# JonathonLuiten/PReMVOS

Hardware: AMD Instinct MI355X
Metric: frames/sec (proposal+refine+flow) on 480p DAVIS frames (higher is better)
Workload: dtype f32

## Files before the change

premvos_amd/_lib.py:

```python
from __future__ import annotations

import ctypes as C
import os

import torch

from . import build as _build

_LIB = None
ABI_VERSION = 21

ACT_NONE, ACT_RELU, ACT_LEAKY, ACT_SIGMOID = 0, 1, 2, 3
MASK_BBOX_SLABS = 16
ACT_SPLIT8_BF16 = 0x200
OUT_NHWC, OUT_PIXSHUF2 = 0, 1
PREC_F32, PREC_BF16, PREC_BF16X3 = 0, 1, 3
PRECISIONS = {"fp32": PREC_F32, "bf16": PREC_BF16, "bf16x3": PREC_BF16X3}


class ConvDesc(C.Structure):
    _fields_ = [
        ("inp", C.c_void_p), ("wgt", C.c_void_p), ("bias", C.c_void_p), ("res", C.c_void_p),
        ("out", C.c_void_p),
        ("n", C.c_int32), ("h", C.c_int32), ("w", C.c_int32), ("cin", C.c_int32),
# ... 96 lines not shown
    "premvos_track_gt_scores_f64": [_vp, _vp, _vp, _i32, _i32, _vp, C.c_double, _vp, _vp, _vp, _vp, _vp, _vp],
    "premvos_track_combine_f64": [_vp, _i32, _i32, _i32, _vp, C.c_int64, _vp, _i32, _vp, _vp, _vp, _vp, _vp, _vp, _vp],
    "premvos_viz_scores_u8": [_vp, _i32, _i32, _vp, _vp, _i32, _vp, _vp, C.c_int64, _vp, _i32, _vp, _vp, C.c_int64, _vp, _vp],
    "premvos_reid_max_distance_f64": [_vp, _i32, _vp, C.c_int64, _vp, _vp, _vp],
    "premvos_davis_counts_u8":[_vp, _vp, _i32, _i32, _i32, _vp, _i32, _i32, _vp, _vp, _vp],
    "premvos_bits_overlap_i32": [_vp, _i32, C.c_int64, C.c_int64, _vp, _vp, _i32, _vp, C.c_int64, _vp, C.c_int64, _vp],
    "premvos_prewarp_reid_f64": [_vp, _vp, _i32, _i32, _vp, _vp, _i32, _vp, _vp, _vp, _vp, _vp],
    "premvos_prewarp_chain_f64": [_vp, C.c_int64, _vp, C.c_int64, _vp, _vp, _vp, _vp, _vp, _vp, _i32, _i32, _vp, _vp, _vp, _vp, _i32, _vp, _vp,
                                  _vp, _vp],
    "premvos_prewarp_paint_bits_u8": [_vp, _i32, C.c_int64, C.c_int64, _vp, _vp, _vp, _vp, _vp, _i32, _vp, _vp, _i32, _i32, _i32, _vp, _vp,
                                      _i32, _vp, _vp],
    "premvos_prewarp_negatives_i32": [_vp, _i32, C.c_int64, C.c_int64, _i32, _i32, _i32, _i32, _vp, _i32, _vp, _vp, _vp, _vp],
    "premvos_prewarp_gather_neg_u8": [_vp, _i32, C.c_int64, _i32, _i32, _i32, _i32, _vp, _vp, _vp, _vp],
    "premvos_prewarp_chain_neg_f64": [_vp, C.c_int64, _vp, C.c_int64, _vp, _vp, _vp, _vp, _vp, _vp, _i32, _i32, _i32, _vp, _vp, _vp, _vp, _i32,
                                      _vp, _vp, _vp, _vp],
    "premvos_prewarp_paint_neg_bits_u8": [_vp, _i32, C.c_int64, C.c_int64, _vp, _vp, _vp, _vp, _vp, _i32, _vp, _vp, _i32, _i32, _i32, _i32, _vp,
                                          _vp, _i32, _vp, _vp],
    "premvos_mask_warp_pack_bits_u8": [_vp, _i32, _i32, _i32, _vp, _vp, _vp, _vp, _vp, _i32, _i32, _vp, _vp, C.c_int64, _vp],
    "premvos_idmap_vote_u8": [_vp, _i32, C.c_int64, C.c_int64, _vp, _vp, _vp, _vp],
    "premvos_crf_unary_labels_f32": [_vp, _i32, _i32, _i32, _i32, _f32, _vp, _vp, _vp, _vp],
    "premvos_crf_norm_f32": [_vp, _i32, _i32, _i32, _f32, _f32, _i32, _vp, _vp],
    "premvos_crf_step_f32": [_vp, _vp, _vp, _vp, _vp, _i32, _i32, _i32, _i32, _f32, _i32, _f32, _f32, _f32, _i32, _f32, _vp, _vp],
    "premvos_crf_argmax_u8": [_vp, _i32, _i32, _i32, _i32, _vp, _vp, _vp, _vp],
}


POST_SIGNATURES = {
    "premvos_cc_dilate_u8": [_vp, _i32, _i32, _i32, _i32, _i32, _vp, _vp],
    "premvos_cc_label_i32": [_vp, C.c_int64, _i32, _i32, _vp, _vp],
    "premvos_cc_keep_largest_u8": [_vp, _vp, _i32, _i32, _i32, _i32, _vp, _vp, _vp, _vp, _vp],
}


class FrameFiles(C.Structure):
    _fields_ = [("flo_path", C.c_char_p), ("flow", C.c_void_p), ("flow_row_stride", C.c_int64), ("h", C.c_int32), ("w", C.c_int32),
                ("boxes", C.c_void_p * 2), ("probs", C.c_void_p * 2), ("count", C.c_int32 * 2), ("scale", C.c_float),
                ("json_path", C.c_char_p * 4), ("conf", C.c_void_p), ("rle_pool", C.c_void_p), ("rle_offsets", C.c_void_p)]


class PremvosError(RuntimeError):
    pass


def lib_path() -> str:
    return _build.LIB


def load():
    global _LIB
    if _LIB is not None:
        return _LIB
    path = _build.LIB
    stale = None
    try:
        if _build.needs_build():
            import fcntl
            with open(os.path.join(os.path.dirname(path), ".build.lock"), "w") as lock:
                fcntl.flock(lock, fcntl.LOCK_EX)
                if _build.needs_build():
                    _build.build_lib()
    except Exception as e:
        if not os.path.exists(path):
            raise PremvosError(
                f"libpremvos_hip.so is missing and could not be built ({e}); the HIP path has no fallback") from e
        stale = e
    lib = C.CDLL(path)
    lib.premvos_last_error.restype = C.c_char_p
    lib.premvos_last_error.argtypes = []
    lib.premvos_abi_version.restype = C.c_int
    lib.premvos_abi_version.argtypes = []
    if lib.premvos_abi_version() != ABI_VERSION:
        raise PremvosError(f"{path} has ABI version {lib.premvos_abi_version()}, this package binds version {ABI_VERSION}"
                           + (f" (rebuilding failed: {stale})" if stale else "") + "; rebuild with python -m premvos_amd.build")
    if stale is not None:
        import warnings
        warnings.warn(f"libpremvos_hip.so is older than its sources and could not be rebuilt ({stale}); using it as is")
    for name, argtypes in list(SIGNATURES.items()) + list(POST_SIGNATURES.items()):
        fn = getattr(lib, name)
        fn.argtypes = argtypes
        fn.restype = C.c_int
    lib.premvos_conv2d_workspace_bytes.argtypes = [C.POINTER(ConvDesc)]
    lib.premvos_conv2d_workspace_bytes.restype = C.c_int64
    lib.premvos_crc32c_host.argtypes = [_vp, C.c_int64]
    lib.premvos_crc32c_host.restype = C.c_uint32
    lib.premvos_refine_output_workspace_bytes.argtypes = [_i32, _i32, _i32, _i32]
    lib.premvos_refine_output_workspace_bytes.restype = C.c_int64
    lib.premvos_rle_counts_to_string_host.argtypes = [_vp, C.c_int64, _vp, C.c_int64]
    lib.premvos_rle_counts_to_string_host.restype = C.c_int64
    lib.premvos_rle_strings_host.argtypes = [_vp, _vp, _i32, C.c_int64, _vp, C.c_int64, _vp]
    lib.premvos_rle_strings_host.restype = C.c_int64
    lib.premvos_write_frame_files_host.argtypes = [C.POINTER(FrameFiles)]
    lib.premvos_write_frame_files_host.restype = C.c_int
    lib.premvos_format_floats_host.argtypes = [_vp, C.c_int64, _i32, _vp, C.c_int64]
    lib.premvos_format_floats_host.restype = C.c_int
    lib.premvos_rle_workspace_bytes.argtypes = [_i32, _i32, _i32]
    lib.premvos_rle_workspace_bytes.restype = C.c_int64
    lib.premvos_jpeg_workspace_bytes.argtypes = [_vp]
    lib.premvos_jpeg_workspace_bytes.restype = C.c_int64
    lib.premvos_dwconv3x3_variant.argtypes = [_i32] * 10
    lib.premvos_dwconv3x3_variant.restype = C.c_int
    _LIB = lib
    return lib


def check(rc: int, what: str = ""):
    if rc != 0:
        raise PremvosError(f"{what} failed ({rc}): {load().premvos_last_error().decode()}")


def current_stream() -> int:
# ... 16 lines not shown
```

premvos_amd/csrc/refine_ops.hip:

```cpp
#include "common.h"

#pragma clang fp contract(off)

namespace {

inline int grid_for(long total, int per_block = 256, int cap = 1 << 22) {
  long g = (total + per_block - 1) / per_block;
  return (int)(g < 1 ? 1 : g > cap ? cap : g);
}

__device__ inline void tf_lerp(int d, float scale, int in_size, int* lo, int* hi, float* t) {
  const float s = (float)d * scale;
  const float f = floorf(s);
  *lo = (int)f;
  const int c = (int)ceilf(s);
  *hi = c < in_size - 1 ? c : in_size - 1;
  *t = s - f;
}

__global__ __launch_bounds__(256) void refine_input_kernel(const uint8_t* __restrict__ frame, int H, int W,
                                                           const float* __restrict__ boxes,
                                                           const int* __restrict__ count, int P, int S,
                                                           float* __restrict__ out, int* __restrict__ crops) {
  const long total = (long)P * S * S;
  const float mean[3] = {0.485f, 0.456f, 0.406f}, stdv[3] = {0.229f, 0.224f, 0.225f};
  const int n = *count < P ? *count : P;
  for (long idx = (long)blockIdx.x * 256 + threadIdx.x; idx < total; idx += (long)gridDim.x * 256) {
    const int x = idx % S, y = (idx / S) % S, p = idx / ((long)S * S);
    float4 o = make_float4(0.f, 0.f, 0.f, 0.f);
    if (p < n) {
      const float* b = boxes + p * 4;
      const int by0 = (int)rintf(b[0]), bx0 = (int)rintf(b[1]), by1 = (int)rintf(b[2]), bx1 = (int)rintf(b[3]);
      const int cy0 = by0 - 50 > 0 ? by0 - 50 : 0, cx0 = bx0 - 50 > 0 ? bx0 - 50 : 0;
// ... 217 lines not shown
        if constexpr (PRE_RELU)
          v[cx] = make_float4(ok ? fmaxf(t.x, 0.f) : 0.f, ok ? fmaxf(t.y, 0.f) : 0.f, ok ? fmaxf(t.z, 0.f) : 0.f, ok ? fmaxf(t.w, 0.f) : 0.f);
        else
          v[cx] = make_float4(ok ? t.x : 0.f, ok ? t.y : 0.f, ok ? t.z : 0.f, ok ? t.w : 0.f);
      }
#pragma unroll
      for (int o = 0; o < TR; ++o) {
        const int kj = j - o * STRIDE;
        if (kj < 0 || kj > 2) continue;
#pragma unroll
        for (int q = 0; q < TW; ++q)
#pragma unroll
          for (int i = 0; i < 3; ++i) {
            const float4 a = v[q * STRIDE + i], kk = k[kj * 3 + i];
            acc[o][q].x += a.x * kk.x; acc[o][q].y += a.y * kk.y; acc[o][q].z += a.z * kk.z; acc[o][q].w += a.w * kk.w;
          }
        if (kj == 2 && oy0 + o * dil < ho) {
          float* orow = out + (((long)b * ho + oy0 + o * dil) * wo) * out_ps;
#pragma unroll
          for (int q = 0; q < TW; ++q) {
            if (ox0 + q * dil >= wo) break;
            float4 r = acc[o][q];
            if ((act & 0xff) == PREMVOS_ACT_RELU) {
              r.x = fmaxf(r.x, 0.f); r.y = fmaxf(r.y, 0.f); r.z = fmaxf(r.z, 0.f); r.w = fmaxf(r.w, 0.f);
            }
            store_unit(orow + (long)(ox0 + q * dil) * out_ps, cg, r, act);
          }
        }
      }
    }
  }
}

__global__ __launch_bounds__(256) void resize_bilinear_kernel(const float* __restrict__ in, int in_ps, int n, int h,
                                                              int w, int c4, float* __restrict__ out, int out_ps,
                                                              int ho, int wo, int align) {
  const long total = (long)n * ho * wo * c4;
  const float sy = (align && ho > 1) ? (float)(h - 1) / (float)(ho - 1) : (float)h / (float)ho;
  const float sx = (align && wo > 1) ? (float)(w - 1) / (float)(wo - 1) : (float)w / (float)wo;
  for (long idx = (long)blockIdx.x * 256 + threadIdx.x; idx < total; idx += (long)gridDim.x * 256) {
    const int cg = idx % c4;
    const long pix = idx / c4;
    const int ox = pix % wo, oy = (pix / wo) % ho, b = pix / ((long)wo * ho);
    int ylo, yhi, xlo, xhi;
    float ty, tx;
    tf_lerp(oy, sy, h, &ylo, &yhi, &ty);
    tf_lerp(ox, sx, w, &xlo, &xhi, &tx);
    const float* base = in + (long)b * h * w * in_ps + cg * 4;
    const float4 tl = *reinterpret_cast<const float4*>(base + ((long)ylo * w + xlo) * in_ps);
    const float4 tr = *reinterpret_cast<const float4*>(base + ((long)ylo * w + xhi) * in_ps);
    const float4 bl = *reinterpret_cast<const float4*>(base + ((long)yhi * w + xlo) * in_ps);
    const float4 br = *reinterpret_cast<const float4*>(base + ((long)yhi * w + xhi) * in_ps);
    float4 o;
    float top, bot;
    top = tl.x + (tr.x - tl.x) * tx; bot = bl.x + (br.x - bl.x) * tx; o.x = top + (bot - top) * ty;
    top = tl.y + (tr.y - tl.y) * tx; bot = bl.y + (br.y - bl.y) * tx; o.y = top + (bot - top) * ty;
    top = tl.z + (tr.z - tl.z) * tx; bot = bl.z + (br.z - bl.z) * tx; o.z = top + (bot - top) * ty;
    top = tl.w + (tr.w - tl.w) * tx; bot = bl.w + (br.w - bl.w) * tx; o.w = top + (bot - top) * ty;
    *reinterpret_cast<float4*>(out + pix * out_ps + cg * 4) = o;
  }
}

__global__ __launch_bounds__(256) void broadcast_kernel(const float* __restrict__ in, int in_ps, int n, int hw, int c4,
                                                        float* __restrict__ out, int out_ps) {
  const long total = (long)n * hw * c4;
  for (long idx = (long)blockIdx.x * 256 + threadIdx.x; idx < total; idx += (long)gridDim.x * 256) {
    const int cg = idx % c4;
    const long pix = idx / c4;
    const int b = pix / hw;
    *reinterpret_cast<float4*>(out + pix * out_ps + cg * 4) =
        *reinterpret_cast<const float4*>(in + (long)b * in_ps + cg * 4);
  }
}

__global__ __launch_bounds__(256) void seg_softmax_kernel(const float* __restrict__ logits, int ps, int P, int lh,
                                                          int lw, int S, float* __restrict__ prob,
                                                          uint8_t* __restrict__ cls) {
  const long total = (long)P * S * S;
  const float sy = (float)lh / (float)S, sx = (float)lw / (float)S;
  for (long idx = (long)blockIdx.x * 256 + threadIdx.x; idx < total; idx += (long)gridDim.x * 256) {
    const int x = idx % S, y = (idx / S) % S, p = idx / ((long)S * S);
    int ylo, yhi, xlo, xhi;
    float ty, tx;
    tf_lerp(y, sy, lh, &ylo, &yhi, &ty);
    tf_lerp(x, sx, lw, &xlo, &xhi, &tx);
    const float* base = logits + (long)p * lh * lw * ps;
    float l[2];
    for (int ch = 0; ch < 2; ++ch) {
      const float tl = base[((long)ylo * lw + xlo) * ps + ch], tr = base[((long)ylo * lw + xhi) * ps + ch];
      const float bl = base[((long)yhi * lw + xlo) * ps + ch], br = base[((long)yhi * lw + xhi) * ps + ch];
      const float top = tl + (tr - tl) * tx, bot = bl + (br - bl) * tx;
      l[ch] = top + (bot - top) * ty;
// ... 253 lines not shown
#define PV_DW_ROW(PR, ST)                                                                                                   \
  hipLaunchKernelGGL((dwconv3x3_row_kernel<PR, ST, 4>), g, dim3(256), 0, s, in, in_ps, n, h, w, c4, wgt, bias, out, out_ps, ho, wo, \
                     pt, pl, act, c_pad)
    if (v.pre_relu && v.stride == 1) PV_DW_ROW(true, 1);
    else if (v.pre_relu) PV_DW_ROW(true, 2);
    else if (v.stride == 1) PV_DW_ROW(false, 1);
    else PV_DW_ROW(false, 2);
#undef PV_DW_ROW
    return premvos::check_launch("dwconv3x3_row");
  }
  const long total = (long)n * ho * wo * c4;
  if (v.pre_relu)
    hipLaunchKernelGGL(dwconv3x3_kernel<true>, dim3(grid_for(total)), dim3(256), 0, s, in, in_ps, n, h, w, c4,
                       wgt, bias, out, out_ps, ho, wo, stride, dilation, pt, pl, act, c_pad);
  else
    hipLaunchKernelGGL(dwconv3x3_kernel<false>, dim3(grid_for(total)), dim3(256), 0, s, in, in_ps, n, h, w, c4,
                       wgt, bias, out, out_ps, ho, wo, stride, dilation, pt, pl, act, c_pad);
  return premvos::check_launch("dwconv3x3");
}

extern "C" int premvos_resize_bilinear_f32(const float* in, int32_t in_ps, int32_t n, int32_t h, int32_t w, int32_t c,
                                           float* out, int32_t out_ps, int32_t ho, int32_t wo, int32_t align_corners,
                                           void* stream) {
  PV_REQUIRE(in && out, "resize_bilinear: null pointer");
  PV_REQUIRE(n > 0 && h > 0 && w > 0 && c > 0 && ho > 0 && wo > 0, "resize_bilinear: bad dims");
  PV_REQUIRE(c % 4 == 0 && in_ps % 4 == 0 && out_ps % 4 == 0 && in_ps >= c && out_ps >= c,
             "resize_bilinear: C and strides must be multiples of 4");
  PV_REQUIRE(premvos::aligned16(in) && premvos::aligned16(out), "resize_bilinear: pointers must be 16-byte aligned");
  hipLaunchKernelGGL(resize_bilinear_kernel, dim3(grid_for((long)n * ho * wo * (c / 4))), dim3(256), 0,
                     static_cast<hipStream_t>(stream), in, in_ps, n, h, w, c / 4, out, out_ps, ho, wo, align_corners);
  return premvos::check_launch("resize_bilinear");
}

extern "C" int premvos_broadcast_pixel_f32(const float* in, int32_t in_ps, int32_t n, int32_t c, float* out,
                                           int32_t out_ps, int32_t h, int32_t w, void* stream) {
  PV_REQUIRE(in && out, "broadcast_pixel: null pointer");
  PV_REQUIRE(n > 0 && c > 0 && h > 0 && w > 0, "broadcast_pixel: bad dims");
  PV_REQUIRE(c % 4 == 0 && in_ps % 4 == 0 && out_ps % 4 == 0 && in_ps >= c && out_ps >= c,
             "broadcast_pixel: C and strides must be multiples of 4");
  PV_REQUIRE(premvos::aligned16(in) && premvos::aligned16(out), "broadcast_pixel: pointers must be 16-byte aligned");
  hipLaunchKernelGGL(broadcast_kernel, dim3(grid_for((long)n * h * w * (c / 4))), dim3(256), 0,
                     static_cast<hipStream_t>(stream), in, in_ps, n, h * w, c / 4, out, out_ps);
  return premvos::check_launch("broadcast_pixel");
}

extern "C" int64_t premvos_refine_output_workspace_bytes(int32_t max_boxes, int32_t size, int32_t h, int32_t w) {
  const long nblk = ((long)h * w + UNCROP_PIX - 1) / UNCROP_PIX;
  return (int64_t)max_boxes * size * size * (sizeof(float) + 1) + (int64_t)max_boxes * nblk * sizeof(double) + 256;
}

namespace {

struct OutputWorkspace {
  double* partial;
  float* prob;
  uint8_t* cls;
  int nblk;
};

inline OutputWorkspace output_workspace(void* workspace, int max_boxes, int size, int h, int w) {
  OutputWorkspace o;
  o.nblk = (int)(((long)h * w + UNCROP_PIX - 1) / UNCROP_PIX);
  char* ws = static_cast<char*>(workspace);
  o.partial = reinterpret_cast<double*>(ws);
  o.prob = reinterpret_cast<float*>(ws + (((long)max_boxes * o.nblk * sizeof(double) + 255) / 256) * 256);
  o.cls = reinterpret_cast<uint8_t*>(o.prob + (long)max_boxes * size * size);
// ... 71 lines not shown
```

premvos_amd/refinement/model.py:

```python
from __future__ import annotations

import os
from typing import Dict, List, Optional, Tuple

import torch

from .. import _lib, arena, ops
from ..ops import ACT_NONE, ACT_RELU, NHWC
from ..plan import LaunchPlan
from . import tta as tta_mod

INPUT_SIZE = 385
EPS_BACKBONE, EPS_HEAD = 1e-3, 1e-5
ATROUS_RATES = (6, 12, 18)
BLOCKS = (
    ("entry_flow/block1", (128, 128, 128), "conv", False, 1, 2),
    ("entry_flow/block2", (256, 256, 256), "conv", False, 1, 2),
    ("entry_flow/block3", (728, 728, 728), "conv", False, 1, 2),
    ("middle_flow/block1", (728, 728, 728), "sum", False, 16, 1),
    ("exit_flow/block1", (728, 1024, 1024), "conv", False, 1, 2),
    ("exit_flow/block2", (1536, 1536, 2048), "none", True, 1, 1),
)
DECODER_SKIP = "entry_flow/block2/unit_1/xception_module/separable_conv2"

# ... 54 lines not shown
        def alloc(n, h, w, c) -> NHWC:
            ps = (c + 3) // 4 * 4
            return NHWC(A.alloc(n, h, w, ps, "f32", pooled=ps == c), c=c)

        def release(v: Optional[NHWC]):
            if v is not None:
                A.release(v)

        split_pw = net.precision == "bf16x3" and os.environ.get("PREMVOS_BF16X3_SPLIT", "1") != "0"
        self.split_pw = split_pw
        S8 = net.packed_s8

        def alloc_s8(n, h, w, c) -> NHWC:
            assert c % 8 == 0
            return NHWC(A.alloc(n, h, w, c, "s8"), c=c, layout="s8")

        scope = {"tag": ""}

        def conv(x, name, out, out_s8=None, **kw):
            self.conv(scope["tag"] + name, x, (S8 if x.layout == "s8" else PK)[name], out, out_s8, **kw)

        def dwconv(x: NHWC, name: str, out: NHWC, stride=1, rate=1, pre_relu=False, act=ACT_NONE):
            k = DW[name]
            assert x.c == k.c and out.c == k.c and x.layout == "f32"
            flags = act | (_lib.ACT_SPLIT8_BF16 if out.layout == "s8" else 0)

            def f(x=x, out=out, k=k):
                _lib.check(lib.premvos_dwconv3x3_f32(x.ptr, x.ps, x.n, x.h, x.w, x.c, k.wgt.data_ptr(),
                                                     k.bias.data_ptr(), k.c_pad, out.ptr, out.ps, out.h, out.w, stride,
                                                     rate, rate, rate, int(pre_relu), flags, _lib.current_stream()),
                           "dwconv3x3")
            self.add(f"dw:{scope['tag']}{name}", f)
            self.dw_bytes[f"dw:{scope['tag']}{name}"] = 4.0 * k.c * (x.n * x.h * x.w + out.n * out.h * out.w)

        def alloc_mid(n, h, w, c, name=None):
            return alloc_s8(n, h, w, c) if split_pw and (name is None or name in S8) else alloc(n, h, w, c)

        S = INPUT_SIZE
        self.frames = A.side((G, H, W, 3), torch.uint8)
        NG = 1 if packed else G
        self.boxes_g = A.side((NG, PF, 4), torch.float32)
        self.count = A.side((G,), torch.int32)
        self.crops = A.side((NG, PF, 4), torch.int32)
        self.frame, self.boxes = self.frames[0], self.boxes_g[0]
        self.net_in = alloc(P, S, S, 4)

        def mk_input():
            if packed:
                for g, off, n in self.layout:
                    _lib.check(lib.premvos_refine_input_u8(self.frames[g].data_ptr(), H, W, self.boxes_g[0, off:].data_ptr(),
                                                           self.count[g:].data_ptr(), n, S, self.net_in.images(off, n).ptr,
                                                           self.crops[0, off:].data_ptr(), _lib.current_stream()), "refine_input")
                return
            for g in range(G):
                _lib.check(lib.premvos_refine_input_u8(self.frames[g].data_ptr(), H, W, self.boxes_g[g].data_ptr(),
                                                       self.count[g:].data_ptr(), PF, S,
                                                       self.net_in.images(g * PF, PF).ptr, self.crops[g].data_ptr(),
                                                       _lib.current_stream()), "refine_input")
        self.add("refine_input", mk_input)

        def body(net_in: NHWC, P: int, S: int, tag: str = "", named: bool = True) -> NHWC:
            scope["tag"] = tag
            h1 = ops.out_size(S, 3, 2, 1, 1)
            c11 = alloc(P, h1, h1, 32)
            conv(net_in, "entry_flow/conv1_1", c11, stride=(2, 2), pad=(1, 1), act=ACT_RELU)
            if net_in is not self.net_in:
# ... 41 lines not shown
                        if f"{prefix}/separable_conv{i}" == DECODER_SKIP:
                            skip_feat = cur
                        else:
                            release(cur)
                    cur = o
                if sc is not None:
                    release(sc)
                release(inp)
                x = cur
            feat = x
            if named:
                self.xception_out = feat
            fh = feat.h

            cat = alloc_mid(P, fh, fh, 1280)
            cat8 = cat.layout == "s8"
            gp = alloc(P, 1, 1, 2048)
            self.add(tag + "gap", lambda i=feat, o=gp: _lib.check(lib.premvos_global_avgpool_f32(
                i.ptr, i.ps, i.n, i.h * i.w, i.c, o.ptr, o.ps, _lib.current_stream()), "gap"))
            ip = alloc(P, 1, 1, 256)
            conv(gp, "image_pooling", ip, act=ACT_RELU)
            release(gp)
            bc = alloc(P, fh, fh, 256) if cat8 else cat.slice(0, 256)
            self.add(tag + "broadcast", lambda i=ip, o=bc: _lib.check(lib.premvos_broadcast_pixel_f32(
                i.ptr, i.ps, i.n, 256, o.ptr, o.ps, o.h, o.w, _lib.current_stream()), "broadcast"))
            release(ip)
            if cat8:
                self.add(f"split8:{tag}image_pooling", lambda i=bc, o=cat.slice(0, 256): ops.split8(i, o))
                release(bc)
                conv(x8, "aspp0", None, cat.slice(256, 256), act=ACT_RELU)
                release(x8)
            else:
                conv(feat, "aspp0", cat.slice(256, 256), act=ACT_RELU)
            for i, r in enumerate(ATROUS_RATES, 1):
                t = alloc_mid(P, fh, fh, 2048)
                dwconv(feat, f"aspp{i}_depthwise", t, rate=r, act=ACT_RELU)
                if cat8:
                    conv(t, f"aspp{i}_pointwise", None, cat.slice(256 * (i + 1), 256), act=ACT_RELU)
                else:
                    conv(t, f"aspp{i}_pointwise", cat.slice(256 * (i + 1), 256), act=ACT_RELU)
                release(t)
            if not named:
                release(feat)
            aspp = alloc(P, fh, fh, 256)
            conv(cat, "concat_projection", aspp, act=ACT_RELU)
            release(cat)
            if named:
                self.aspp_out = aspp

            dh = int((float(S) - 1.0) * 0.25 + 1.0)
            assert skip_feat is not None and skip_feat.h == dh
            dcat = alloc(P, dh, dh, 304)
            self.add(tag + "resize_aspp", lambda i=aspp, o=dcat.slice(0, 256): _lib.check(lib.premvos_resize_bilinear_f32(
                i.ptr, i.ps, i.n, i.h, i.w, 256, o.ptr, o.ps, o.h, o.w, 1, _lib.current_stream()), "resize"))
            if not named:
                release(aspp)
            conv(skip_feat, "decoder/feature_projection0", dcat.slice(256, 48), act=ACT_RELU)
            release(skip_feat)
            d = dcat
            for j in (0, 1):
                t = alloc_mid(P, dh, dh, d.c, f"decoder/decoder_conv{j}_pointwise")
                dwconv(d, f"decoder/decoder_conv{j}_depthwise", t, act=ACT_RELU)
                release(d)
                o = alloc(P, dh, dh, 256)
                conv(t, f"decoder/decoder_conv{j}_pointwise", o, act=ACT_RELU)
                release(t)
                d = o
            logits = alloc(P, dh, dh, 2)
            conv(d, "logits/features", logits)
            if named:
                self.decoder_out = d
            else:
                release(d)
            scope["tag"] = ""
            return logits

        tta = net.tta
        self.member_logits: List[NHWC] = []
        if tta is None:
            self.logits = body(self.net_in, P, S)
            self.member_logits.append(self.logits)
        else:
            self.logits = None
            nb = 2 if tta.flip else 1
            for scale in tta.scales:
                Ss, L = tta_mod.scale_dimension(S, scale), tta_mod.scale_dimension(S, max(1.0, scale) / 4.0)
                if Ss == S and nb == 1:
                    x = self.net_in
                else:
                    x = alloc(P * nb, Ss, Ss, 4)
                    self.add(f"tta_input:{Ss}", lambda o=x, Ss=Ss: _lib.check(lib.premvos_refine_tta_input_f32(
                        self.net_in.ptr, P, S, o.ptr, Ss, nb - 1, _lib.current_stream()), "refine_tta_input"))
                lg = body(x, P * nb, Ss, tag=f"tta{Ss}/", named=False)
                if lg.h != L:
                    assert lg.h < L and lg.ps == 4
# ... 160 lines not shown
```

Before: 54.26.

## Fuse ASPP atrous depthwise convs and decoder upsample into depthwise kernels

Adds a multirate depthwise kernel that computes all three ASPP atrous depthwise convolutions in one pass over the feature map, plus a lattice variant for small maps. It also adds a decoder depthwise kernel that bilinearly upsamples the ASPP output on the fly instead of writing a resized tensor first. The aim is fewer launches and less global memory traffic on the refinement network tail. In exchange it adds new code paths, higher register pressure, and all three ASPP temporaries must be live at the same time.

```diff
diff --git a/include/premvos_refine_hip.h b/include/premvos_refine_hip.h
--- /dev/null
+++ b/include/premvos_refine_hip.h
@@ -0,0 +1,21 @@
+#ifndef PREMVOS_REFINE_HIP_H
+#define PREMVOS_REFINE_HIP_H
+
+#include <stdint.h>
+
+#ifdef __cplusplus
+extern "C" {
+#endif
+
+int premvos_dwconv3x3_upsrc_f32(const float* src, int32_t src_ps, int32_t hs, int32_t ws, int32_t c_up, const float* in, int32_t in_ps,
+                                int32_t n, int32_t h, int32_t w, int32_t c, const float* wgt, const float* bias, int32_t c_pad, float* out,
+                                int32_t out_ps, int32_t act, void* stream);
+
+int premvos_dwconv3x3_multirate_f32(const float* in, int32_t in_ps, int32_t n, int32_t h, int32_t w, int32_t c, int32_t c_pad,
+                                    int32_t n_rates, const int32_t* rates, const float* const* wgt, const float* const* bias,
+                                    float* const* out, const int32_t* out_ps, int32_t act, void* stream);
+
+#ifdef __cplusplus
+}
+#endif
+#endif
diff --git a/premvos_amd/_lib.py b/premvos_amd/_lib.py
--- a/premvos_amd/_lib.py
+++ b/premvos_amd/_lib.py
@@ -152,6 +152,18 @@
 }
 
 
+REFINE_SIGNATURES = {
+    "premvos_dwconv3x3_upsrc_f32": [_vp, _i32, _i32, _i32, _i32, _vp, _i32, _i32, _i32, _i32, _i32, _vp, _vp, _i32, _vp, _i32, _i32, _vp],
+    "premvos_dwconv3x3_multirate_f32": [_vp, _i32, _i32, _i32, _i32, _i32, _i32, _i32, _vp, _vp, _vp, _vp, _vp, _i32, _vp],
+}
+
+
+def multirate_args(rates, wgts, biases, outs, out_ps):
+    n = len(rates)
+    assert 1 <= n <= 3 and len(wgts) == len(biases) == len(outs) == len(out_ps) == n
+    return ((C.c_int32 * n)(*rates), (C.c_void_p * n)(*wgts), (C.c_void_p * n)(*biases), (C.c_void_p * n)(*outs), (C.c_int32 * n)(*out_ps))
+
+
 class FrameFiles(C.Structure):
     _fields_ = [("flo_path", C.c_char_p), ("flow", C.c_void_p), ("flow_row_stride", C.c_int64), ("h", C.c_int32), ("w", C.c_int32),
                 ("boxes", C.c_void_p * 2), ("probs", C.c_void_p * 2), ("count", C.c_int32 * 2), ("scale", C.c_float),
@@ -195,7 +207,7 @@
     if stale is not None:
         import warnings
         warnings.warn(f"libpremvos_hip.so is older than its sources and could not be rebuilt ({stale}); using it as is")
-    for name, argtypes in list(SIGNATURES.items()) + list(POST_SIGNATURES.items()):
+    for name, argtypes in list(SIGNATURES.items()) + list(POST_SIGNATURES.items()) + list(REFINE_SIGNATURES.items()):
         fn = getattr(lib, name)
         fn.argtypes = argtypes
         fn.restype = C.c_int
diff --git a/premvos_amd/csrc/refine_ops.hip b/premvos_amd/csrc/refine_ops.hip
--- a/premvos_amd/csrc/refine_ops.hip
+++ b/premvos_amd/csrc/refine_ops.hip
@@ -1,4 +1,7 @@
+#include <utility>
+
 #include "common.h"
+#include "../../include/premvos_refine_hip.h"
 
 #pragma clang fp contract(off)
 
@@ -282,12 +285,24 @@
   }
 }
 
+__device__ __forceinline__ float resize_scale(int in_size, int out_size, int align) {
+  return (align && out_size > 1) ? (float)(in_size - 1) / (float)(out_size - 1) : (float)in_size / (float)out_size;
+}
+
+__device__ __forceinline__ float4 lerp4(const float4 a, const float4 b, const float t) {
+  return make_float4(a.x + (b.x - a.x) * t, a.y + (b.y - a.y) * t, a.z + (b.z - a.z) * t, a.w + (b.w - a.w) * t);
+}
+
+__device__ __forceinline__ float4 bilerp4(const float4 tl, const float4 tr, const float4 bl, const float4 br, const float tx,
+                                          const float ty) {
+  return lerp4(lerp4(tl, tr, tx), lerp4(bl, br, tx), ty);
+}
+
 __global__ __launch_bounds__(256) void resize_bilinear_kernel(const float* __restrict__ in, int in_ps, int n, int h,
                                                               int w, int c4, float* __restrict__ out, int out_ps,
                                                               int ho, int wo, int align) {
   const long total = (long)n * ho * wo * c4;
-  const float sy = (align && ho > 1) ? (float)(h - 1) / (float)(ho - 1) : (float)h / (float)ho;
-  const float sx = (align && wo > 1) ? (float)(w - 1) / (float)(wo - 1) : (float)w / (float)wo;
+  const float sy = resize_scale(h, ho, align), sx = resize_scale(w, wo, align);
   for (long idx = (long)blockIdx.x * 256 + threadIdx.x; idx < total; idx += (long)gridDim.x * 256) {
     const int cg = idx % c4;
     const long pix = idx / c4;
@@ -301,13 +316,298 @@
     const float4 tr = *reinterpret_cast<const float4*>(base + ((long)ylo * w + xhi) * in_ps);
     const float4 bl = *reinterpret_cast<const float4*>(base + ((long)yhi * w + xlo) * in_ps);
     const float4 br = *reinterpret_cast<const float4*>(base + ((long)yhi * w + xhi) * in_ps);
-    float4 o;
-    float top, bot;
-    top = tl.x + (tr.x - tl.x) * tx; bot = bl.x + (br.x - bl.x) * tx; o.x = top + (bot - top) * ty;
-    top = tl.y + (tr.y - tl.y) * tx; bot = bl.y + (br.y - bl.y) * tx; o.y = top + (bot - top) * ty;
-    top = tl.z + (tr.z - tl.z) * tx; bot = bl.z + (br.z - bl.z) * tx; o.z = top + (bot - top) * ty;
-    top = tl.w + (tr.w - tl.w) * tx; bot = bl.w + (br.w - bl.w) * tx; o.w = top + (bot - top) * ty;
-    *reinterpret_cast<float4*>(out + pix * out_ps + cg * 4) = o;
+    *reinterpret_cast<float4*>(out + pix * out_ps + cg * 4) = bilerp4(tl, tr, bl, br, tx, ty);
+  }
+}
+
+template <class F, int... I>
+__device__ __forceinline__ void static_for_impl(F&& f, std::integer_sequence<int, I...>) {
+  (f(std::integral_constant<int, I>{}), ...);
+}
+template <int N, class F>
+__device__ __forceinline__ void static_for(F&& f) {
+  static_for_impl(f, std::make_integer_sequence<int, N>{});
+}
+constexpr int f4_lo(int m) { return m < 0 ? 0 : 1 + m / 4; }
+constexpr int f4_hi(int m) { return f4_lo(m) + (((m + 4) & 3) ? 1 : 0); }
+constexpr float f4_t(int m) { return (float)((m + 4) & 3) * 0.25f; }
+
+__global__ __launch_bounds__(256) void dwconv3x3_upsrc_kernel(const float* __restrict__ src, int src_ps, int hs, int ws, int cup4,
+                                                              const float* __restrict__ in, int in_ps, int n, int h, int w,
+                                                              int c4, const float* __restrict__ wgt,
+                                                              const float* __restrict__ bias, float* __restrict__ out,
+                                                              int out_ps, int act, int cpad, int up_blocks) {
+  constexpr int TW = 4, TR = 8, NCOL = TW + 2, NROW = TR + 2;
+  const int xt = (w + TW - 1) / TW, yt = (h + TR - 1) / TR;
+  const bool up = (int)blockIdx.x < up_blocks;
+  const int ncg = up ? cup4 : c4 - cup4;
+  const long idx = (long)(up ? blockIdx.x : blockIdx.x - up_blocks) * 256 + threadIdx.x;
+  if (idx >= (long)n * yt * xt * ncg) return;
+  const int lcg = idx % ncg;
+  long t = idx / ncg;
+  const int tx = t % xt;
+  t /= xt;
+  const int ty = t % yt, b = t / yt;
+  const int cg = up ? lcg : cup4 + lcg;
+  const int ox0 = tx * TW, oy0 = ty * TR, ix0 = ox0 - 1, iy0 = oy0 - 1;
+  float4 k[9];
+#pragma unroll
+  for (int i = 0; i < 9; ++i) k[i] = *reinterpret_cast<const float4*>(wgt + (long)i * cpad + cg * 4);
+  float4 bv = make_float4(0.f, 0.f, 0.f, 0.f);
+  if (bias != nullptr) bv = *reinterpret_cast<const float4*>(bias + cg * 4);
+  float4 acc[TR][TW];
+#pragma unroll
+  for (int o = 0; o < TR; ++o)
+#pragma unroll
+    for (int q = 0; q < TW; ++q) acc[o][q] = bv;
+  auto row_ok = [&](int j) { return (unsigned)(iy0 + j) < (unsigned)h; };
+  auto col_ok = [&](int cx) { return (unsigned)(ix0 + cx) < (unsigned)w; };
+  auto store_row = [&](int o) __attribute__((always_inline)) {
+    if (oy0 + o >= h) return;
+    float* orow = out + (((long)b * h + oy0 + o) * w) * out_ps;
+#pragma unroll
+    for (int q = 0; q < TW; ++q) {
+      if (ox0 + q >= w) break;
+      float4 r = acc[o][q];
+      if ((act & 0xff) == PREMVOS_ACT_RELU) {
+        r.x = fmaxf(r.x, 0.f); r.y = fmaxf(r.y, 0.f); r.z = fmaxf(r.z, 0.f); r.w = fmaxf(r.w, 0.f);
+      }
+      store_unit(orow + (long)(ox0 + q) * out_ps, cg, r, act);
+    }
+  };
+  auto consume = [&](auto J, const float4* v) __attribute__((always_inline)) {
+    constexpr int j = decltype(J)::value;
+#pragma unroll
+    for (int o = 0; o < TR; ++o) {
+      const int kj = j - o;
+      if (kj < 0 || kj > 2) continue;
+#pragma unroll
+      for (int q = 0; q < TW; ++q)
+#pragma unroll
+        for (int i = 0; i < 3; ++i) {
+          const float4 a = v[q + i], kk = k[kj * 3 + i];
+          acc[o][q].x += a.x * kk.x; acc[o][q].y += a.y * kk.y; acc[o][q].z += a.z * kk.z; acc[o][q].w += a.w * kk.w;
+        }
+      if (kj == 2) store_row(o);
+    }
+  };
+  auto masked = [&](int j, int cx, const float4 s) {
+    const bool ok = row_ok(j) && col_ok(cx);
+    return make_float4(ok ? s.x : 0.f, ok ? s.y : 0.f, ok ? s.z : 0.f, ok ? s.w : 0.f);
+  };
+
+  if (!up) {
+    const float* imgp = in + ((long)b * h * w) * in_ps + lcg * 4;
+    auto load_row = [&](int j, float4* v) {
+      const float* rowp = imgp + ((long)(iy0 + j) * w) * in_ps;
+#pragma unroll
+      for (int cx = 0; cx < NCOL; ++cx)
+        if (row_ok(j) && col_ok(cx)) v[cx] = *reinterpret_cast<const float4*>(rowp + (long)(ix0 + cx) * in_ps);
+    };
+    float4 vbuf[2][NCOL];
+    load_row(0, vbuf[0]);
+    static_for<NROW>([&](auto J) __attribute__((always_inline)) {
+      constexpr int j = decltype(J)::value;
+      if (j + 1 < NROW) load_row(j + 1, vbuf[(j + 1) & 1]);
+      float4 v[NCOL];
+#pragma unroll
+      for (int cx = 0; cx < NCOL; ++cx) {
+        const bool ok = row_ok(j) && col_ok(cx);
+        const float4& s = vbuf[j & 1][cx];
+        v[cx] = make_float4(ok ? s.x : 0.f, ok ? s.y : 0.f, ok ? s.z : 0.f, ok ? s.w : 0.f);
+      }
+      consume(J, v);
+    });
+    return;
+  }
+
+  const float* simg = src + ((long)b * hs * ws) * src_ps + cg * 4;
+  {
+    constexpr int PR = 4, PC = 3;
+    const int sy0 = oy0 / 4 - 1, sx0 = ox0 / 4 - 1;
+    float4 p[PR][PC], hb[PR][NCOL];
+    auto load_patch_row = [&](int r) {
+#pragma unroll
+      for (int c = 0; c < PC; ++c) {
+        p[r][c] = premvos::arbitrary4();
+        if ((unsigned)(sy0 + r) < (unsigned)hs && (unsigned)(sx0 + c) < (unsigned)ws)
+          p[r][c] = *reinterpret_cast<const float4*>(simg + ((long)(sy0 + r) * ws + sx0 + c) * src_ps);
+      }
+    };
+    auto blend_row = [&](int r) {
+#pragma unroll
+      for (int cx = 0; cx < NCOL; ++cx)
+        hb[r][cx] = lerp4(p[r][f4_lo(cx - 1)], p[r][f4_hi(cx - 1)], f4_t(cx - 1));
+    };
+    load_patch_row(0), load_patch_row(1);
+    static_for<NROW>([&](auto J) __attribute__((always_inline)) {
+      constexpr int j = decltype(J)::value, m = j - 1;
+      if constexpr (j == 0) blend_row(0), blend_row(1), load_patch_row(2);
+      if constexpr (j == 2) blend_row(2);
+      if constexpr (j == 4) load_patch_row(3);
+      if constexpr (j == 6) blend_row(3);
+      float4 v[NCOL];
+#pragma unroll
+      for (int cx = 0; cx < NCOL; ++cx) v[cx] = masked(j, cx, lerp4(hb[f4_lo(m)][cx], hb[f4_hi(m)][cx], f4_t(m)));
+      consume(J, v);
+    });
+  }
+}
+
+__global__ __launch_bounds__(256) void dwconv3x3_upsrc_pixel_kernel(const float* __restrict__ src, int src_ps, int hs, int ws,
+                                                                    int cup4, const float* __restrict__ in, int in_ps, int n, int h,
+                                                                    int w, int c4, const float* __restrict__ wgt,
+                                                                    const float* __restrict__ bias, float* __restrict__ out,
+                                                                    int out_ps, int act, int cpad) {
+  const long total = (long)n * h * w * c4;
+  const float sy = resize_scale(hs, h, 1), sx = resize_scale(ws, w, 1);
+  for (long idx = (long)blockIdx.x * 256 + threadIdx.x; idx < total; idx += (long)gridDim.x * 256) {
+    const int cg = idx % c4;
+    const long pix = idx / c4;
+    const int ox = pix % w, oy = (pix / w) % h, b = pix / ((long)w * h);
+    const bool up = cg < cup4;
+    const float* simg = src + ((long)b * hs * ws) * src_ps + cg * 4;
+    const float* img = in + ((long)b * h * w) * in_ps + (cg - cup4) * 4;
+    float4 acc = make_float4(0.f, 0.f, 0.f, 0.f);
+    if (bias != nullptr) acc = *reinterpret_cast<const float4*>(bias + cg * 4);
+#pragma unroll
+    for (int j = 0; j < 3; ++j) {
+      const int iy = oy - 1 + j;
+      if ((unsigned)iy >= (unsigned)h) continue;
+#pragma unroll
+      for (int i = 0; i < 3; ++i) {
+        const int ix = ox - 1 + i;
+        if ((unsigned)ix >= (unsigned)w) continue;
+        float4 v;
+        if (up) {
+          int ylo, yhi, xlo, xhi;
+          float fy, fx;
+          tf_lerp(iy, sy, hs, &ylo, &yhi, &fy);
+          tf_lerp(ix, sx, ws, &xlo, &xhi, &fx);
+          v = bilerp4(*reinterpret_cast<const float4*>(simg + ((long)ylo * ws + xlo) * src_ps),
+                      *reinterpret_cast<const float4*>(simg + ((long)ylo * ws + xhi) * src_ps),
+                      *reinterpret_cast<const float4*>(simg + ((long)yhi * ws + xlo) * src_ps),
+                      *reinterpret_cast<const float4*>(simg + ((long)yhi * ws + xhi) * src_ps), fx, fy);
+        } else {
+          v = *reinterpret_cast<const float4*>(img + ((long)iy * w + ix) * in_ps);
+        }
+        const float4 kk = *reinterpret_cast<const float4*>(wgt + (long)(j * 3 + i) * cpad + cg * 4);
+        acc.x += v.x * kk.x; acc.y += v.y * kk.y; acc.z += v.z * kk.z; acc.w += v.w * kk.w;
+      }
+    }
+    if ((act & 0xff) == PREMVOS_ACT_RELU) {
+      acc.x = fmaxf(acc.x, 0.f); acc.y = fmaxf(acc.y, 0.f); acc.z = fmaxf(acc.z, 0.f); acc.w = fmaxf(acc.w, 0.f);
+    }
+    store_unit(out + pix * out_ps, cg, acc, act);
+  }
+}
+
+struct DwMultiRate {
+  int rate[3];
+  const float* wgt[3];
+  const float* bias[3];
+  float* out[3];
+  int out_ps[3];
+};
+
+template <int NR>
+__global__ __launch_bounds__(256) void dwconv3x3_multirate_kernel(const float* __restrict__ in, int in_ps, int n, int h, int w,
+                                                                  int c4, const DwMultiRate a, int act, int cpad) {
+  const long total = (long)n * h * w * c4;
+  for (long idx = (long)blockIdx.x * 256 + threadIdx.x; idx < total; idx += (long)gridDim.x * 256) {
+    const int cg = idx % c4;
+    const long pix = idx / c4;
+    const int ox = pix % w, oy = (pix / w) % h, b = pix / ((long)w * h);
+    const float* img = in + ((long)b * h * w) * in_ps + cg * 4;
+    const float4 ctr = *reinterpret_cast<const float4*>(img + ((long)oy * w + ox) * in_ps);
+    float4 raw[NR][9];
+#pragma unroll
+    for (int r = 0; r < NR; ++r)
+#pragma unroll
+      for (int tap = 0; tap < 9; ++tap) {
+        if (tap == 4) continue;
+        const int iy = oy + (tap / 3 - 1) * a.rate[r], ix = ox + (tap % 3 - 1) * a.rate[r];
+        raw[r][tap] = premvos::arbitrary4();
+        if ((unsigned)iy < (unsigned)h && (unsigned)ix < (unsigned)w)
+          raw[r][tap] = *reinterpret_cast<const float4*>(img + ((long)iy * w + ix) * in_ps);
+      }
+#pragma unroll
+    for (int r = 0; r < NR; ++r) {
+      float4 acc = make_float4(0.f, 0.f, 0.f, 0.f);
+      if (a.bias[r] != nullptr) acc = *reinterpret_cast<const float4*>(a.bias[r] + cg * 4);
+#pragma unroll
+      for (int tap = 0; tap < 9; ++tap) {
+        const int iy = oy + (tap / 3 - 1) * a.rate[r], ix = ox + (tap % 3 - 1) * a.rate[r];
+        if (tap != 4 && !((unsigned)iy < (unsigned)h && (unsigned)ix < (unsigned)w)) continue;
+        const float4 v = tap == 4 ? ctr : raw[r][tap];
+        const float4 kk = *reinterpret_cast<const float4*>(a.wgt[r] + (long)tap * cpad + cg * 4);
+        acc.x += v.x * kk.x; acc.y += v.y * kk.y; acc.z += v.z * kk.z; acc.w += v.w * kk.w;
+      }
+      if ((act & 0xff) == PREMVOS_ACT_RELU) {
+        acc.x = fmaxf(acc.x, 0.f); acc.y = fmaxf(acc.y, 0.f); acc.z = fmaxf(acc.z, 0.f); acc.w = fmaxf(acc.w, 0.f);
+      }
+      store_unit(a.out[r] + pix * a.out_ps[r], cg, acc, act);
+    }
+  }
+}
+
+constexpr int DW_LATTICE = 5;
+__global__ __launch_bounds__(256) void dwconv3x3_lattice3_kernel(const float* __restrict__ in, int in_ps, int n, int h, int w,
+                                                                 int c4, const DwMultiRate a, int act, int cpad) {
+  constexpr int NL = DW_LATTICE;
+  const int d = a.rate[0];
+  const long total = (long)n * d * d * c4;
+  for (long idx = (long)blockIdx.x * 256 + threadIdx.x; idx < total; idx += (long)gridDim.x * 256) {
+    const int cg = idx % c4;
+    long t = idx / c4;
+    const int rx = t % d;
+    t /= d;
+    const int ry = t % d, b = t / d;
+    const float* img = in + ((long)b * h * w) * in_ps + cg * 4;
+    auto inside = [&](int i, int j) { return ry + i * d < h && rx + j * d < w; };
+    float4 v[NL][NL];
+#pragma unroll
+    for (int i = 0; i < NL; ++i)
+#pragma unroll
+      for (int j = 0; j < NL; ++j) {
+        v[i][j] = premvos::arbitrary4();
+        if (inside(i, j)) v[i][j] = *reinterpret_cast<const float4*>(img + ((long)(ry + i * d) * w + rx + j * d) * in_ps);
+      }
+#pragma unroll
+    for (int i = 0; i < NL; ++i)
+#pragma unroll
+      for (int j = 0; j < NL; ++j) {
+        const bool ok = inside(i, j);
+        const float4 s = v[i][j];
+        v[i][j] = make_float4(ok ? s.x : 0.f, ok ? s.y : 0.f, ok ? s.z : 0.f, ok ? s.w : 0.f);
+      }
+#pragma unroll
+    for (int r = 0; r < 3; ++r) {
+      const int step = r + 1;
+      float4 k[9];
+#pragma unroll
+      for (int tap = 0; tap < 9; ++tap) k[tap] = *reinterpret_cast<const float4*>(a.wgt[r] + (long)tap * cpad + cg * 4);
+      float4 bv = make_float4(0.f, 0.f, 0.f, 0.f);
+      if (a.bias[r] != nullptr) bv = *reinterpret_cast<const float4*>(a.bias[r] + cg * 4);
+#pragma unroll
+      for (int i = 0; i < NL; ++i)
+#pragma unroll
+        for (int j = 0; j < NL; ++j) {
+          float4 acc = bv;
+#pragma unroll
+          for (int tap = 0; tap < 9; ++tap) {
+            const int ii = i + (tap / 3 - 1) * step, jj = j + (tap % 3 - 1) * step;
+            if (ii < 0 || ii >= NL || jj < 0 || jj >= NL) continue;
+            const float4 s = v[ii][jj], kk = k[tap];
+            acc.x += s.x * kk.x; acc.y += s.y * kk.y; acc.z += s.z * kk.z; acc.w += s.w * kk.w;
+          }
+          if ((act & 0xff) == PREMVOS_ACT_RELU) {
+            acc.x = fmaxf(acc.x, 0.f); acc.y = fmaxf(acc.y, 0.f); acc.z = fmaxf(acc.z, 0.f); acc.w = fmaxf(acc.w, 0.f);
+          }
+          if (inside(i, j))
+            store_unit(a.out[r] + (((long)b * h + ry + i * d) * w + rx + j * d) * a.out_ps[r], cg, acc, act);
+        }
+    }
   }
 }
 
@@ -627,6 +927,73 @@
   return premvos::check_launch("resize_bilinear");
 }
 
+extern "C" int premvos_dwconv3x3_upsrc_f32(const float* src, int32_t src_ps, int32_t hs, int32_t ws, int32_t c_up, const float* in,
+                                           int32_t in_ps, int32_t n, int32_t h, int32_t w, int32_t c, const float* wgt,
+                                           const float* bias, int32_t c_pad, float* out, int32_t out_ps, int32_t act, void* stream) {
+  PV_REQUIRE(src && wgt && out, "dwconv3x3_upsrc: null pointer");
+  PV_REQUIRE(n > 0 && h > 0 && w > 0 && hs > 0 && ws > 0 && c > 0 && c_pad >= c && c_pad % 4 == 0, "dwconv3x3_upsrc: bad dims");
+  PV_REQUIRE(c_up > 0 && c_up % 4 == 0 && c_up <= c_pad, "dwconv3x3_upsrc: c_up must be a multiple of 4 in (0, c_pad]");
+  PV_REQUIRE(c_up == c_pad || in != nullptr, "dwconv3x3_upsrc: null pointer");
+  PV_REQUIRE(src_ps % 4 == 0 && in_ps % 4 == 0 && out_ps % 4 == 0 && src_ps >= c_up && out_ps >= c_pad &&
+                 (c_up == c_pad || in_ps >= c_pad - c_up),
+             "dwconv3x3_upsrc: channel count / strides must be padded to multiples of 4");
+  PV_REQUIRE(premvos::aligned16(src) && premvos::aligned16(in) && premvos::aligned16(out) && premvos::aligned16(wgt) &&
+                 (bias == nullptr || premvos::aligned16(bias)),
+             "dwconv3x3_upsrc: pointers must be 16-byte aligned");
+  PV_REQUIRE(act == PREMVOS_ACT_NONE || act == PREMVOS_ACT_RELU, "dwconv3x3_upsrc: bad activation (fp32 output only)");
+  const int c4 = c_pad / 4, cup4 = c_up / 4;
+  const long tiles = (long)n * ((h + 7) / 8) * ((w + 3) / 4);
+  const long up_blocks = (tiles * cup4 + 255) / 256, in_blocks = (tiles * (c4 - cup4) + 255) / 256;
+  PV_REQUIRE(up_blocks + in_blocks <= (1L << 22), "dwconv3x3_upsrc: too many tiles for one launch");
+  const dim3 g((unsigned)(up_blocks + in_blocks));
+  hipStream_t s = static_cast<hipStream_t>(stream);
+  if (hs > 1 && ws > 1 && h - 1 == 4 * (hs - 1) && w - 1 == 4 * (ws - 1))
+    hipLaunchKernelGGL(dwconv3x3_upsrc_kernel, g, dim3(256), 0, s, src, src_ps, hs, ws, cup4, in, in_ps, n, h, w, c4, wgt, bias, out,
+                       out_ps, act, c_pad, (int)up_blocks);
+  else
+    hipLaunchKernelGGL(dwconv3x3_upsrc_pixel_kernel, dim3(grid_for((long)n * h * w * c4)), dim3(256), 0, s, src, src_ps, hs, ws, cup4,
+                       in, in_ps, n, h, w, c4, wgt, bias, out, out_ps, act, c_pad);
+  return premvos::check_launch("dwconv3x3_upsrc");
+}
+
+extern "C" int premvos_dwconv3x3_multirate_f32(const float* in, int32_t in_ps, int32_t n, int32_t h, int32_t w, int32_t c,
+                                               int32_t c_pad, int32_t n_rates, const int32_t* rates, const float* const* wgt,
+                                               const float* const* bias, float* const* out, const int32_t* out_ps, int32_t act,
+                                               void* stream) {
+  PV_REQUIRE(in && rates && wgt && bias && out && out_ps, "dwconv3x3_multirate: null pointer");
+  PV_REQUIRE(n_rates >= 1 && n_rates <= 3, "dwconv3x3_multirate: 1 to 3 rates");
+  PV_REQUIRE(c > 0, "dwconv3x3_multirate: bad dims");
+  if (dw_check_shape(n, h, w, c_pad, h, w, 1, 1, act) != 0) return -1;
+  PV_REQUIRE(c_pad >= c && in_ps % 4 == 0 && in_ps >= c_pad, "dwconv3x3_multirate: channel count / strides must be padded to multiples of 4");
+  PV_REQUIRE(premvos::aligned16(in), "dwconv3x3_multirate: pointers must be 16-byte aligned");
+  DwMultiRate a{};
+  for (int r = 0; r < n_rates; ++r) {
+    PV_REQUIRE(rates[r] > 0, "dwconv3x3_multirate: bad dims");
+    PV_REQUIRE(wgt[r] && out[r], "dwconv3x3_multirate: null pointer");
+    PV_REQUIRE(out_ps[r] % 4 == 0 && out_ps[r] >= c_pad, "dwconv3x3_multirate: channel count / strides must be padded to multiples of 4");
+    PV_REQUIRE(premvos::aligned16(wgt[r]) && premvos::aligned16(out[r]) && (bias[r] == nullptr || premvos::aligned16(bias[r])),
+               "dwconv3x3_multirate: pointers must be 16-byte aligned");
+    PV_REQUIRE(!(act & PREMVOS_ACT_SPLIT8_BF16) || (out_ps[r] % 8 == 0 && (reinterpret_cast<uintptr_t>(out[r]) & 31u) == 0),
+               "dwconv3x3_multirate: an S8 output needs out_ps %% 8 == 0 and a 32-byte aligned channel window");
+    a.rate[r] = rates[r], a.wgt[r] = wgt[r], a.bias[r] = bias[r], a.out[r] = out[r], a.out_ps[r] = out_ps[r];
+  }
+  const int c4 = c_pad / 4;
+  if ((act & PREMVOS_ACT_SPLIT8_BF16) && c4 % 2 == 0) act |= DW_PAIRED;
+  hipStream_t s = static_cast<hipStream_t>(stream);
+  const long d = a.rate[0];
+  if (n_rates == 3 && a.rate[1] == 2 * d && a.rate[2] == 3 * d && h <= DW_LATTICE * d && w <= DW_LATTICE * d && d <= h &&
+      d <= w) {
+    hipLaunchKernelGGL(dwconv3x3_lattice3_kernel, dim3(grid_for((long)n * d * d * c4)), dim3(256), 0, s, in, in_ps, n, h, w, c4, a, act,
+                       c_pad);
+    return premvos::check_launch("dwconv3x3_multirate");
+  }
+  const dim3 g(grid_for((long)n * h * w * c4));
+  if (n_rates == 3) hipLaunchKernelGGL(dwconv3x3_multirate_kernel<3>, g, dim3(256), 0, s, in, in_ps, n, h, w, c4, a, act, c_pad);
+  else if (n_rates == 2) hipLaunchKernelGGL(dwconv3x3_multirate_kernel<2>, g, dim3(256), 0, s, in, in_ps, n, h, w, c4, a, act, c_pad);
+  else hipLaunchKernelGGL(dwconv3x3_multirate_kernel<1>, g, dim3(256), 0, s, in, in_ps, n, h, w, c4, a, act, c_pad);
+  return premvos::check_launch("dwconv3x3_multirate");
+}
+
 extern "C" int premvos_broadcast_pixel_f32(const float* in, int32_t in_ps, int32_t n, int32_t c, float* out,
                                            int32_t out_ps, int32_t h, int32_t w, void* stream) {
   PV_REQUIRE(in && out, "broadcast_pixel: null pointer");
diff --git a/premvos_amd/refinement/model.py b/premvos_amd/refinement/model.py
--- a/premvos_amd/refinement/model.py
+++ b/premvos_amd/refinement/model.py
@@ -110,6 +110,36 @@
                            "dwconv3x3")
             self.add(f"dw:{scope['tag']}{name}", f)
             self.dw_bytes[f"dw:{scope['tag']}{name}"] = 4.0 * k.c * (x.n * x.h * x.w + out.n * out.h * out.w)
+
+        tail = os.environ.get("PREMVOS_REFINE_TAIL", "fused")
+        assert tail in ("fused", "steps", "multirate", "upsrc"), tail
+        fuse_aspp, fuse_dec = not split_pw and tail in ("fused", "multirate"), not split_pw and tail in ("fused", "upsrc")
+        self.tail = (fuse_aspp, fuse_dec)
+
+        def dwconv_multirate(x: NHWC, names: List[str], outs: List[NHWC], rates, step: str, act=ACT_NONE):
+            ks = [DW[nm] for nm in names]
+            assert all(k.c == x.c and o.c == x.c and o.layout == "f32" for k, o in zip(ks, outs)) and x.layout == "f32"
+            rates = list(rates)
+
+            def f(x=x, ks=ks, outs=list(outs)):
+                args = _lib.multirate_args(rates, [k.wgt.data_ptr() for k in ks], [k.bias.data_ptr() for k in ks],
+                                           [o.ptr for o in outs], [o.ps for o in outs])
+                _lib.check(lib.premvos_dwconv3x3_multirate_f32(x.ptr, x.ps, x.n, x.h, x.w, x.c, ks[0].c_pad, len(ks), *args, act,
+                                                               _lib.current_stream()), "dwconv3x3_multirate")
+            self.add(f"dw:{scope['tag']}{step}", f)
+            self.dw_bytes[f"dw:{scope['tag']}{step}"] = 4.0 * x.c * x.n * x.h * x.w * (1 + len(ks))
+
+        def dwconv_upsrc(src: NHWC, x: NHWC, name: str, out: NHWC, act=ACT_NONE):
+            k = DW[name]
+            assert src.c + x.c == k.c == out.c and src.c % 4 == 0 and src.n == x.n == out.n and (x.h, x.w) == (out.h, out.w)
+            assert src.layout == x.layout == out.layout == "f32"
+
+            def f(src=src, x=x, out=out, k=k):
+                _lib.check(lib.premvos_dwconv3x3_upsrc_f32(src.ptr, src.ps, src.h, src.w, src.c, x.ptr, x.ps, x.n, x.h, x.w, k.c,
+                                                           k.wgt.data_ptr(), k.bias.data_ptr(), k.c_pad, out.ptr, out.ps, act,
+                                                           _lib.current_stream()), "dwconv3x3_upsrc")
+            self.add(f"dw:{scope['tag']}{name}", f)
+            self.dw_bytes[f"dw:{scope['tag']}{name}"] = 4.0 * (src.c * src.n * src.h * src.w + x.c * x.n * x.h * x.w + k.c * out.n * out.h * out.w)
 
         def alloc_mid(n, h, w, c, name=None):
             return alloc_s8(n, h, w, c) if split_pw and (name is None or name in S8) else alloc(n, h, w, c)
@@ -217,9 +247,15 @@
                 release(x8)
             else:
                 conv(feat, "aspp0", cat.slice(256, 256), act=ACT_RELU)
+            ts = None
+            if fuse_aspp:
+                ts = [alloc(P, fh, fh, 2048) for _ in ATROUS_RATES]
+                dwconv_multirate(feat, [f"aspp{i}_depthwise" for i in range(1, len(ATROUS_RATES) + 1)], ts, ATROUS_RATES,
+                                 "aspp_depthwise", act=ACT_RELU)
             for i, r in enumerate(ATROUS_RATES, 1):
-                t = alloc_mid(P, fh, fh, 2048)
-                dwconv(feat, f"aspp{i}_depthwise", t, rate=r, act=ACT_RELU)
+                t = ts[i - 1] if ts else alloc_mid(P, fh, fh, 2048)
+                if ts is None:
+                    dwconv(feat, f"aspp{i}_depthwise", t, rate=r, act=ACT_RELU)
                 if cat8:
                     conv(t, f"aspp{i}_pointwise", None, cat.slice(256 * (i + 1), 256), act=ACT_RELU)
                 else:
@@ -236,16 +272,22 @@
             dh = int((float(S) - 1.0) * 0.25 + 1.0)
             assert skip_feat is not None and skip_feat.h == dh
             dcat = alloc(P, dh, dh, 304)
-            self.add(tag + "resize_aspp", lambda i=aspp, o=dcat.slice(0, 256): _lib.check(lib.premvos_resize_bilinear_f32(
-                i.ptr, i.ps, i.n, i.h, i.w, 256, o.ptr, o.ps, o.h, o.w, 1, _lib.current_stream()), "resize"))
-            if not named:
-                release(aspp)
+            if not fuse_dec:
+                self.add(tag + "resize_aspp", lambda i=aspp, o=dcat.slice(0, 256): _lib.check(lib.premvos_resize_bilinear_f32(
+                    i.ptr, i.ps, i.n, i.h, i.w, 256, o.ptr, o.ps, o.h, o.w, 1, _lib.current_stream()), "resize"))
+                if not named:
+                    release(aspp)
             conv(skip_feat, "decoder/feature_projection0", dcat.slice(256, 48), act=ACT_RELU)
             release(skip_feat)
             d = dcat
             for j in (0, 1):
                 t = alloc_mid(P, dh, dh, d.c, f"decoder/decoder_conv{j}_pointwise")
-                dwconv(d, f"decoder/decoder_conv{j}_depthwise", t, act=ACT_RELU)
+                if j == 0 and fuse_dec:
+                    dwconv_upsrc(aspp, dcat.slice(256, 48), "decoder/decoder_conv0_depthwise", t, act=ACT_RELU)
+                    if not named:
+                        release(aspp)
+                else:
+                    dwconv(d, f"decoder/decoder_conv{j}_depthwise", t, act=ACT_RELU)
                 release(d)
                 o = alloc(P, dh, dh, 256)
                 conv(t, f"decoder/decoder_conv{j}_pointwise", o, act=ACT_RELU)
```

After: 54.77, median of 6. About the same (+0.9%).
